# pengsongyou/openscene

Measured on AMD Instinct MI355X. Metric: active voxels/sec MinkUNet18A fwd+bwd @2cm ScanNet; per-point query ms, higher is better.
Workload: dtype f32 (bf16x6 split-precision MFMA, fp32 accumulate); 1 GPU; ScanNet distillation step (configs[2]): MinkUNet18A, 768-d head, 1 synthetic S100k scene/GPU (100999 voxels on rank 0, 2 cm), training-mode BN; timed = coordinate+kernel maps, forward, cosine loss, backward, gradient all-reduce, Adam step; arch=MinkUNet18A, feature_dim=768, voxels_rank0=100999, parallelism=dp1

## Files before the change

### openscene_amd/csrc/spconv_ws.hip

```cpp
#include "common.h"
#include "split.h"
#include "pairlist.h"
#include "epilogue.h"

namespace osn {

constexpr int WS_NG = 4;
constexpr int WS_CH = 32 * WS_NG;

template <int NW, int KS, bool EPI = false>
__global__ __launch_bounds__(256) void spconv_ws_kernel(const float* __restrict__ in, const bf16x8* __restrict__ Wp,
                                                        const int32_t* __restrict__ gsrc, const int32_t* __restrict__ gdst,
                                                        const int32_t* __restrict__ poff, float* __restrict__ partial,
                                                        float* __restrict__ zeros, int n_dst, int K, int cin, int cout, int ns, int ncb, int chunk,
                                                        int direct, const Epi epi) {
    constexpr int NT = 256;
    constexpr int CK = 32 * KS;
    constexpr int LDA = CK + 8;
    constexpr int QPR = CK / 4;
    constexpr int NQ = (32 * QPR + NT - 1) / NT;
    __shared__ __attribute__((aligned(16))) __bf16 stage[2][3][32][LDA];
    __shared__ int sidx[WS_CH], didx[WS_CH];

    const int tid = threadIdx.x, lane = tid & 63;
    const int wave = __builtin_amdgcn_readfirstlane(tid >> 6);
    const int k = blockIdx.y;
    if (blockIdx.x == 0 && blockIdx.y == 0 && blockIdx.z == 0 && tid < 64) zeros[tid] = 0.f;
    const int pk0 = poff[k], pk1 = poff[k + 1];
    const int p0 = pk0 + blockIdx.x * chunk;
    if (p0 >= pk1) return;
    const int np = min(chunk, pk1 - p0);
    const int nsteps = (np + 31) >> 5;
    const int col0 = blockIdx.z * (32 * NW);
    const int cb0 = blockIdx.z * (2 * NW) + 2 * wave;

    for (int e = tid; e < WS_CH; e += NT) {
        sidx[e] = e < np ? gsrc[p0 + e] : 0;
        didx[e] = e < np ? gdst[p0 + e] : -1;
    }
    int q_row[NQ], q_col[NQ];
#pragma unroll
    for (int j = 0; j < NQ; ++j) {
        const int idx = tid + NT * j;
        q_row[j] = (idx / QPR) & 31;
        q_col[j] = (idx % QPR) * 4;
    }
    __syncthreads();

    f32x4 acc[WS_NG][2][2];
#pragma unroll
    for (int g = 0; g < WS_NG; ++g)
#pragma unroll
        for (int h = 0; h < 2; ++h)
#pragma unroll
            for (int nb = 0; nb < 2; ++nb) acc[g][h][nb] = f32x4{0.f, 0.f, 0.f, 0.f};

    float4 P[NQ];
    auto fetch = [&](int g, int s0) {
#pragma unroll
        for (int j = 0; j < NQ; ++j) {
            const unsigned row = unsigned(sidx[32 * g + q_row[j]]);
            const int ch = 32 * s0 + q_col[j];
            const unsigned cu = ch < cin ? unsigned(ch) : 0u;
            P[j] = *reinterpret_cast<const float4*>(in + (uint64_t(row) * unsigned(cin) + cu));
        }
    };
    int buf = 0;
    for (int s0 = 0; s0 < ns; s0 += KS) {
        bf16x8 B[KS][2][3];
        if (wave < NW) {
#pragma unroll
            for (int ks = 0; ks < KS; ++ks)
#pragma unroll
                for (int nb = 0; nb < 2; ++nb) {
                    const bool on = s0 + ks < ns && cb0 + nb < ncb;
                    const unsigned sb = on ? unsigned(s0 + ks) : 0u, cb = on ? unsigned(cb0 + nb) : 0u;
#pragma unroll
                    for (int pl = 0; pl < 3; ++pl) {
                        const unsigned blk = (unsigned(pl * K + k) * unsigned(ns) + sb) * unsigned(ncb) + cb;
                        B[ks][nb][pl] = (Wp + (size_t(blk) << 6))[lane];
                    }
                }
        }
        fetch(0, s0);
#pragma unroll
        for (int g = 0; g < WS_NG; ++g) {
            if (g < nsteps) {
#pragma unroll
                for (int j = 0; j < NQ; ++j) {
                    const bool ok = 32 * s0 + q_col[j] < cin;
                    bf16x4 p1, p2, p3;
                    tl_split4(ok ? P[j] : make_float4(0.f, 0.f, 0.f, 0.f), p1, p2, p3);
                    if (NT * NQ == 32 * QPR || tid + NT * j < 32 * QPR) {
                        *reinterpret_cast<bf16x4*>(&stage[buf][0][q_row[j]][q_col[j]]) = p1;
                        *reinterpret_cast<bf16x4*>(&stage[buf][1][q_row[j]][q_col[j]]) = p2;
                        *reinterpret_cast<bf16x4*>(&stage[buf][2][q_row[j]][q_col[j]]) = p3;
                    }
                }
                if (g + 1 < nsteps) fetch(g + 1, s0);
                __syncthreads();
                if (wave < NW) {
                    const bool half1 = np - 32 * g > 16;
                    const int akq = 8 * (lane >> 4);
#pragma unroll
                    for (int ks = 0; ks < KS; ++ks) {
                        if (s0 + ks < ns) {
                            bf16x8 af[2][3];
#pragma unroll
                            for (int h = 0; h < 2; ++h)
#pragma unroll
                                for (int pl = 0; pl < 3; ++pl)
                                    af[h][pl] = *reinterpret_cast<const bf16x8*>(
                                        &stage[buf][pl][(half1 ? h : 0) * 16 + (lane & 15)][ks * 32 + akq]);
                            auto mfma_half = [&](int h, auto ap, auto bp) {
#pragma unroll
                                for (int nb = 0; nb < 2; ++nb)
                                    acc[g][h][nb] = __builtin_amdgcn_mfma_f32_16x16x32_bf16(B[ks][nb][bp], af[h][ap], acc[g][h][nb], 0, 0, 0);
                            };
                            if (half1) split_products([&](auto ap, auto bp) { mfma_half(0, ap, bp); mfma_half(1, ap, bp); });
                            else split_products([&](auto ap, auto bp) { mfma_half(0, ap, bp); });
                        }
                    }
                }
                buf ^= 1;
            }
        }
    }
    if (wave >= NW) return;
    EpiCols ec[2];
    if constexpr (EPI) {
#pragma unroll
        for (int nb = 0; nb < 2; ++nb) {
            const int col = col0 + 32 * wave + 16 * nb + 4 * (lane >> 4);
            ec[nb] = epi_cols(epi, col < cout ? col : 0);
        }
    }
#pragma unroll
    for (int g = 0; g < WS_NG; ++g) {
        if (g < nsteps) {
#pragma unroll
            for (int h = 0; h < 2; ++h) {
                const int d = didx[32 * g + 16 * h + (lane & 15)];
                if (d >= 0) {
                    float* row = partial + ((direct ? int64_t(0) : int64_t(k) * n_dst) + d) * cout;
#pragma unroll
                    for (int nb = 0; nb < 2; ++nb) {
                        const int col = col0 + 32 * wave + 16 * nb + 4 * (lane >> 4);
                        if (col < cout) {
                            float4 v = make_float4(acc[g][h][nb][0], acc[g][h][nb][1], acc[g][h][nb][2], acc[g][h][nb][3]);
                            if constexpr (EPI) v = epi_apply(epi, ec[nb], v, d, col, cout);
                            *reinterpret_cast<float4*>(row + col) = v;
                        }
                    }
                }
            }
        }
    }
}

constexpr int WS_RED_GROUP = 9;
template <int KT, bool EPI = false>
__global__ __launch_bounds__(256, 8) void spconv_ws_reduce_kernel(const float* __restrict__ partial, const int32_t* __restrict__ nbr,
                                                               const float* __restrict__ zeros, float* __restrict__ out,
                                                               int64_t n_dst, int K, int c4, const Epi epi) {
    const int64_t total = n_dst * c4;
    const int64_t e = int64_t(blockIdx.x) * blockDim.x + threadIdx.x;
    if (e >= total) return;
    const int64_t r = e / c4;
    const int c = int(e - r * c4);
    float4 s = make_float4(0.f, 0.f, 0.f, 0.f);
    if (KT > 0) {
        constexpr int G = KT > 0 && KT % WS_RED_GROUP == 0 ? WS_RED_GROUP : (KT > 0 ? KT : 1);
        static_assert(KT <= 32 && (KT <= 0 || KT % G == 0), "one mask word, whole groups");
        unsigned present = 0;
#pragma unroll
        for (int k = 0; k < KT; ++k) present |= (nbr[int64_t(k) * n_dst + r] >= 0 ? 1u : 0u) << k;
#pragma unroll 1
        for (int k0 = 0; k0 < KT; k0 += G) {
            float4 v[G];
#pragma unroll
            for (int j = 0; j < G; ++j) {
                const float* src = (present >> (k0 + j)) & 1u ? partial + ((int64_t(k0 + j) * n_dst + r) * c4 + c) * 4 : zeros;
                v[j] = *reinterpret_cast<const float4*>(src);
            }
#pragma unroll
            for (int j = 0; j < G; ++j) { s.x += v[j].x; s.y += v[j].y; s.z += v[j].z; s.w += v[j].w; }
        }
    } else {
        for (int k = 0; k < K; ++k) {
            if (nbr[int64_t(k) * n_dst + r] >= 0) {
                const float4 v = *reinterpret_cast<const float4*>(partial + ((int64_t(k) * n_dst + r) * c4 + c) * 4);
                s.x += v.x; s.y += v.y; s.z += v.z; s.w += v.w;
            }
        }
    }
    if constexpr (EPI) s = epi_quad(epi, s, r, 4 * c, 4 * c4);
    reinterpret_cast<float4*>(out)[e] = s;
}

static int ws_waves(int cout) {
    int best = 1, best_pad = 1 << 30;
    for (int nw = 4; nw >= 1; --nw) {
        const int cw = 32 * nw;
        const int pad = int(cdiv(cout, cw)) * cw - cout;
        if (pad < best_pad) { best_pad = pad; best = nw; }
    }
    return best;
}

}

using namespace osn;

extern "C" size_t osn_spconv_fwd_ws_ws_bytes(int64_t n_dst, int K, int cout, int direct) {
    return 256 + (direct ? 0 : size_t(K) * size_t(n_dst > 0 ? n_dst : 0) * size_t(cout) * 4);
}

int osn::spconv_fwd_ws_epi(const float* in, int64_t n_in, const void* Wp, const void* pl, int64_t pl_rows, int swap, int direct,
                           const int32_t* nbr_dst, float* out, int64_t n_dst, int K, int cin, int cout, void* ws, size_t ws_bytes,
                           const Epi& epi, osn_stream_t stream) {
    hipStream_t st = static_cast<hipStream_t>(stream);
    OSN_REQUIRE(n_dst >= 0 && n_dst < (int64_t(1) << 31) && n_in >= 0 && n_in < (int64_t(1) << 31), OSN_E_ARG,
                "osn_spconv_fwd_ws: row counts out of range");
    OSN_REQUIRE(K >= 2 && K <= PL_KMAX && cin >= 4 && (cin & 3) == 0 && cout >= 4 && (cout & 3) == 0, OSN_E_ARG,
                "osn_spconv_fwd_ws: needs 2 <= K <= %d, cin %% 4 == 0, cout %% 4 == 0 (K=%d cin=%d cout=%d)", PL_KMAX, K, cin, cout);
    OSN_REQUIRE(pl_rows == (swap ? n_in : n_dst), OSN_E_ARG,
                "osn_spconv_fwd_ws: the pair arrays are of a map with %lld output rows, this launch writes %lld rows (swap=%d)",
                (long long)pl_rows, (long long)(swap ? n_in : n_dst), swap);
    if (n_dst == 0) return OSN_OK;
    OSN_REQUIRE(in && Wp && pl && (nbr_dst || direct) && out, OSN_E_ARG, "osn_spconv_fwd_ws: null pointer");
    OSN_REQUIRE(aligned16(in) && aligned16(Wp) && aligned16(out) && aligned16(ws), OSN_E_ARG, "osn_spconv_fwd_ws: pointers must be 16-byte aligned");
    const size_t need = osn_spconv_fwd_ws_ws_bytes(n_dst, K, cout, direct);
    OSN_REQUIRE(ws && ws_bytes >= need, OSN_E_WS, "osn_spconv_fwd_ws: workspace %zu < %zu", ws_bytes, need);
    PlView v = pl_view(const_cast<void*>(pl), pl_rows, K, 1);
    const int32_t* gsrc = swap ? v.pout : v.pin;
    const int32_t* gdst = swap ? v.pin : v.pout;
    float* zeros = static_cast<float*>(ws);
    float* partial = reinterpret_cast<float*>(static_cast<char*>(ws) + 256);
    const int nw = ws_waves(cout);
    const int gz = int(cdiv(cout, 32 * nw));
    const int ns = (cin + 31) / 32, ncb = (cout + 15) / 16;
    const int ks = ns <= 4 ? ns : (ns % 4 == 0 ? 4 : (ns % 3 == 0 ? 3 : 4));
    const int64_t pmax = n_in < n_dst ? n_in : n_dst;
    const int chunk = pmax <= 4096 ? 64 : WS_CH;
    const dim3 grid(unsigned(cdiv(pmax, chunk)), unsigned(K), unsigned(gz));
    const bf16x8* wp = static_cast<const bf16x8*>(Wp);
#define OSN_WS2(NW_, KS_)                                                                                              \
    do {                                                                                                               \
        if (direct && epi.mean)                                                                                        \
            hipLaunchKernelGGL((spconv_ws_kernel<NW_, KS_, true>), grid, dim3(256), 0, st, in, wp, gsrc, gdst, v.poff, out, zeros, \
                               int(n_dst), K, cin, cout, ns, ncb, chunk, direct, epi);                                 \
        else                                                                                                           \
            hipLaunchKernelGGL((spconv_ws_kernel<NW_, KS_, false>), grid, dim3(256), 0, st, in, wp, gsrc, gdst, v.poff,  \
                               direct ? out : partial, zeros, int(n_dst), K, cin, cout, ns, ncb, chunk, direct, epi_none()); \
    } while (0)
#define OSN_WS(NW_)                                                                                                    \
    do {                                                                                                               \
        switch (ks) {                                                                                                  \
            case 1: OSN_WS2(NW_, 1); break;                                                                            \
            case 2: OSN_WS2(NW_, 2); break;                                                                            \
            case 3: OSN_WS2(NW_, 3); break;                                                                            \
            default: OSN_WS2(NW_, 4); break;                                                                           \
        }                                                                                                              \
    } while (0)
    switch (nw) {
        case 4: OSN_WS(4); break;
        case 3: OSN_WS(3); break;
        case 2: OSN_WS(2); break;
        default: OSN_WS(1); break;
    }
#undef OSN_WS
#undef OSN_WS2
    if (direct) {
        OSN_LAUNCH_CHECK();
        return OSN_OK;
    }
    const int c4 = cout / 4;
    const dim3 rgrid(unsigned(cdiv(n_dst * c4, 256)));
#define OSN_WSR(KT_)                                                                                                                    \
    do {                                                                                                                                \
        if (epi.mean) hipLaunchKernelGGL((spconv_ws_reduce_kernel<KT_, true>), rgrid, dim3(256), 0, st, partial, nbr_dst, zeros, out, n_dst, K, c4, epi); \
        else hipLaunchKernelGGL((spconv_ws_reduce_kernel<KT_, false>), rgrid, dim3(256), 0, st, partial, nbr_dst, zeros, out, n_dst, K, c4, epi);         \
    } while (0)
    if (K == 27) OSN_WSR(27);
    else if (K == 8) OSN_WSR(8);
    else OSN_WSR(0);
#undef OSN_WSR
    OSN_LAUNCH_CHECK();
    return OSN_OK;
}

extern "C" int osn_spconv_fwd_ws(const float* in, int64_t n_in, const void* Wp, const void* pl, int64_t pl_rows,
                                 int swap, int direct, const int32_t* nbr_dst, float* out, int64_t n_dst, int K, int cin, int cout,
                                 void* ws, size_t ws_bytes, osn_stream_t stream) {
    return spconv_fwd_ws_epi(in, n_in, Wp, pl, pl_rows, swap, direct, nbr_dst, out, n_dst, K, cin, cout, ws, ws_bytes, epi_none(), stream);
}
```

Measured before the change: 12.92 million voxels/s.

## Compact sparse-conv work items and prefetch weights and gathers ahead

Result: no change. 12.99 million voxels/s, median of 6 (+0.5%).

```diff
diff --git a/openscene_amd/csrc/spconv_ws.hip b/openscene_amd/csrc/spconv_ws.hip
--- a/openscene_amd/csrc/spconv_ws.hip
+++ b/openscene_amd/csrc/spconv_ws.hip
@@ -7,6 +7,39 @@
 
 constexpr int WS_NG = 4;
 constexpr int WS_CH = 32 * WS_NG;
+
+#ifndef OSN_WS_PARTS
+#define OSN_WS_PARTS 7
+#endif
+constexpr bool WS_LIVE = (OSN_WS_PARTS & 1) != 0, WS_HOIST = (OSN_WS_PARTS & 2) != 0, WS_CHAIN = (OSN_WS_PARTS & 4) != 0;
+
+__device__ inline bool ws_item(const int32_t* __restrict__ poff, int K, int csh, int item, int lane, int& k, int& p0, int& pk1) {
+    int before = 0;
+    for (int k0 = 0; k0 < K; k0 += 64) {
+        const int kk = k0 + lane;
+        const int a = poff[min(kk, K)], b = poff[min(kk + 1, K)];
+        const int c = (b - a + (1 << csh) - 1) >> csh;
+        int incl = c;
+        incl += __builtin_amdgcn_update_dpp(0, incl, 0x111, 0xf, 0xf, false);
+        incl += __builtin_amdgcn_update_dpp(0, incl, 0x112, 0xf, 0xf, false);
+        incl += __builtin_amdgcn_update_dpp(0, incl, 0x114, 0xf, 0xf, false);
+        incl += __builtin_amdgcn_update_dpp(0, incl, 0x118, 0xf, 0xf, false);
+        incl += __builtin_amdgcn_update_dpp(0, incl, 0x142, 0xa, 0xf, false);
+        incl += __builtin_amdgcn_update_dpp(0, incl, 0x143, 0xc, 0xf, false);
+        incl += before;
+        const int n = __builtin_amdgcn_readfirstlane(__popcll(__ballot(incl <= item)));
+        if (n < 64) {
+            const int cn = __builtin_amdgcn_readlane(c, n), an = __builtin_amdgcn_readlane(a, n);
+            const int j = item - (__builtin_amdgcn_readlane(incl, n) - cn);
+            k = k0 + n;
+            p0 = an + (j << csh);
+            pk1 = __builtin_amdgcn_readlane(b, n);
+            return k < K && j >= 0 && p0 < pk1;
+        }
+        before = __builtin_amdgcn_readlane(incl, 63);
+    }
+    return false;
+}
 
 template <int NW, int KS, bool EPI = false>
 __global__ __launch_bounds__(256) void spconv_ws_kernel(const float* __restrict__ in, const bf16x8* __restrict__ Wp,
@@ -19,24 +52,50 @@
     constexpr int LDA = CK + 8;
     constexpr int QPR = CK / 4;
     constexpr int NQ = (32 * QPR + NT - 1) / NT;
+    static_assert(WS_CH <= NT, "one index pair per thread");
     __shared__ __attribute__((aligned(16))) __bf16 stage[2][3][32][LDA];
     __shared__ int sidx[WS_CH], didx[WS_CH];
 
     const int tid = threadIdx.x, lane = tid & 63;
     const int wave = __builtin_amdgcn_readfirstlane(tid >> 6);
-    const int k = blockIdx.y;
     if (blockIdx.x == 0 && blockIdx.y == 0 && blockIdx.z == 0 && tid < 64) zeros[tid] = 0.f;
-    const int pk0 = poff[k], pk1 = poff[k + 1];
-    const int p0 = pk0 + blockIdx.x * chunk;
-    if (p0 >= pk1) return;
+    int k, p0, pk1;
+    if constexpr (WS_LIVE) {
+        if (!ws_item(poff, K, 31 - __clz(chunk), blockIdx.x, lane, k, p0, pk1)) return;
+    } else {
+        k = blockIdx.y;
+        pk1 = poff[k + 1];
+        p0 = poff[k] + blockIdx.x * chunk;
+        if (p0 >= pk1) return;
+    }
     const int np = min(chunk, pk1 - p0);
     const int nsteps = (np + 31) >> 5;
     const int col0 = blockIdx.z * (32 * NW);
     const int cb0 = blockIdx.z * (2 * NW) + 2 * wave;
 
-    for (int e = tid; e < WS_CH; e += NT) {
-        sidx[e] = e < np ? gsrc[p0 + e] : 0;
-        didx[e] = e < np ? gdst[p0 + e] : -1;
+    const int pe = p0 + min(tid, np - 1);
+    const int src_e = gsrc[pe], dst_e = gdst[pe];
+    bf16x8 B[KS][2][3];
+    auto load_B = [&](int s0) {
+        if (wave < NW) {
+#pragma unroll
+            for (int ks = 0; ks < KS; ++ks)
+#pragma unroll
+                for (int nb = 0; nb < 2; ++nb) {
+                    const bool on = s0 + ks < ns && cb0 + nb < ncb;
+                    const unsigned sb = on ? unsigned(s0 + ks) : 0u, cb = on ? unsigned(cb0 + nb) : 0u;
+#pragma unroll
+                    for (int pl = 0; pl < 3; ++pl) {
+                        const unsigned blk = (unsigned(pl * K + k) * unsigned(ns) + sb) * unsigned(ncb) + cb;
+                        B[ks][nb][pl] = (Wp + (size_t(blk) << 6))[lane];
+                    }
+                }
+        }
+    };
+    if constexpr (WS_HOIST) load_B(0);
+    if (tid < WS_CH) {
+        sidx[tid] = tid < np ? src_e : 0;
+        didx[tid] = tid < np ? dst_e : -1;
     }
     int q_row[NQ], q_col[NQ];
 #pragma unroll
@@ -66,23 +125,10 @@
         }
     };
     int buf = 0;
+    if constexpr (WS_CHAIN) fetch(0, 0);
     for (int s0 = 0; s0 < ns; s0 += KS) {
-        bf16x8 B[KS][2][3];
-        if (wave < NW) {
-#pragma unroll
-            for (int ks = 0; ks < KS; ++ks)
-#pragma unroll
-                for (int nb = 0; nb < 2; ++nb) {
-                    const bool on = s0 + ks < ns && cb0 + nb < ncb;
-                    const unsigned sb = on ? unsigned(s0 + ks) : 0u, cb = on ? unsigned(cb0 + nb) : 0u;
-#pragma unroll
-                    for (int pl = 0; pl < 3; ++pl) {
-                        const unsigned blk = (unsigned(pl * K + k) * unsigned(ns) + sb) * unsigned(ncb) + cb;
-                        B[ks][nb][pl] = (Wp + (size_t(blk) << 6))[lane];
-                    }
-                }
-        }
-        fetch(0, s0);
+        if (!WS_HOIST || s0 > 0) load_B(s0);
+        if constexpr (!WS_CHAIN) fetch(0, s0);
 #pragma unroll
         for (int g = 0; g < WS_NG; ++g) {
             if (g < nsteps) {
@@ -98,6 +144,7 @@
                     }
                 }
                 if (g + 1 < nsteps) fetch(g + 1, s0);
+                else if (WS_CHAIN && s0 + KS < ns) fetch(0, s0 + KS);
                 __syncthreads();
                 if (wave < NW) {
                     const bool half1 = np - 32 * g > 16;
@@ -243,7 +290,9 @@
     const int ks = ns <= 4 ? ns : (ns % 4 == 0 ? 4 : (ns % 3 == 0 ? 3 : 4));
     const int64_t pmax = n_in < n_dst ? n_in : n_dst;
     const int chunk = pmax <= 4096 ? 64 : WS_CH;
-    const dim3 grid(unsigned(cdiv(pmax, chunk)), unsigned(K), unsigned(gz));
+    int64_t items = int64_t(K) * cdiv(pmax > 0 ? pmax : 1, chunk);
+    if (direct && n_dst / chunk + K < items) items = n_dst / chunk + K;
+    const dim3 grid = WS_LIVE ? dim3(unsigned(items), 1u, unsigned(gz)) : dim3(unsigned(cdiv(pmax, chunk)), unsigned(K), unsigned(gz));
     const bf16x8* wp = static_cast<const bf16x8*>(Wp);
 #define OSN_WS2(NW_, KS_)                                                                                              \
     do {                                                                                                               \
```
